# Visual-Behavior/detr-tensorflow

Measured on AMD Instinct MI355X. Metric: images/sec training step, DETR-R50 800x1333 bs=8/GPU, higher is better.
Workload: dtype bf16

## Files before the change

detr-tensorflow_amd/csrc/common.h:

```cpp
#pragma once
#include <hip/hip_runtime.h>
#include <stdint.h>
#include <stdio.h>
#include <stdarg.h>
#include <stdlib.h>

#include "../../include/detr_hip.h"

namespace detr {

void set_error(const char *fmt, ...);

#define DETR_REQUIRE(cond, ...)                 \
    do {                                        \
        if (!(cond)) {                          \
            ::detr::set_error(__VA_ARGS__);     \
            return -1;                          \
        }                                       \
    } while (0)

#define DETR_LAUNCH_CHECK(name)                                                         \
    do {                                                                                \
        hipError_t e__ = hipGetLastError();                                             \
        if (e__ != hipSuccess) {                                                        \
            ::detr::set_error("%s: launch failed: %s", name, hipGetErrorString(e__));   \
            return -2;                                                                  \
        }                                                                               \
    } while (0)

void launch_splitk_reduce(const detr_reduce_desc &r, hipStream_t stream);

constexpr int MIN_WAVES_64X64 = 1;

#if defined(__HIPCC__)
__device__ __forceinline__ void wave_lds_sync() {
    __builtin_amdgcn_fence(__ATOMIC_SEQ_CST, "wavefront");
    __builtin_amdgcn_wave_barrier();
}
__device__ __forceinline__ void lds_barrier() {
    __builtin_amdgcn_fence(__ATOMIC_RELEASE, "workgroup", "local");
    __builtin_amdgcn_s_barrier();
    __builtin_amdgcn_fence(__ATOMIC_ACQUIRE, "workgroup", "local");
}
#endif

enum TuneKey {
    T_GEMM_TILE,
    T_SPLIT_XCD,
    T_GEMM_STREAM,
    T_GEMM_GROUP,
    T_STREAM_SL,
    T_STREAM_NW,
    T_CONV_HALO,
    T_CONV_TILE,
    T_DGRAD_S2_CLASSES,
    T_WGRAD_FUSED,
    T_WGRAD_FUSED_WGS,
    T_WGRAD_TILE,
    T_STEM_ROWS,
    T_ATTN_WAVES,
    T_ATTN_SPLIT,
    T_GEMM_K64,
    T_EPI_WIDE,
    T_SLAB_TS,
    T_GEMM_RING,
// ... 77 lines not shown
```

detr-tensorflow_amd/csrc/optim.hip:

```cpp
#include "common.h"

namespace detr {

__global__ __launch_bounds__(256) void sumsq_segments_kernel(const float *__restrict__ g,
                                                             const int *__restrict__ chunk_tensor,
                                                             const long long *__restrict__ chunk_start,
                                                             const long long *__restrict__ seg_end, int chunk,
                                                             float *__restrict__ sumsq) {
    __shared__ float red[4];
    const int c = blockIdx.x;
    const int t = chunk_tensor[c];
    const long long s0 = chunk_start[c];
    long long s1 = s0 + chunk;
    if (s1 > seg_end[t]) s1 = seg_end[t];
    float acc = 0.f;
    for (long long i = s0 + threadIdx.x; i < s1; i += blockDim.x) {
        const float v = g[i];
        acc += v * v;
    }
    acc = wave_sum(acc);
    if ((threadIdx.x & 63) == 0) red[threadIdx.x >> 6] = acc;
    __syncthreads();
    if (threadIdx.x == 0) sumsq[c] = (red[0] + red[1]) + (red[2] + red[3]);
}

__global__ __launch_bounds__(256) void clip_adam_kernel(float *__restrict__ param, const float *__restrict__ g,
                                                        float *__restrict__ m, float *__restrict__ v,
                                                        const int *__restrict__ chunk_tensor,
                                                        const long long *__restrict__ chunk_start,
                                                        const long long *__restrict__ seg_end,
                                                        const int *__restrict__ tensor_group,
                                                        const float *__restrict__ sumsq,
                                                        const float *__restrict__ hyper, int chunk, int n_chunks) {
    const int c = blockIdx.x;
    const int t = chunk_tensor[c];
    const long long s0 = chunk_start[c];
    long long s1 = s0 + chunk;
    if (s1 > seg_end[t]) s1 = seg_end[t];
    const int grp = tensor_group[t];
    if (grp < 0) return;
    const float lr_t = hyper[grp];
    const float clip = hyper[3], b1 = hyper[4], b2 = hyper[5], eps = hyper[6];
    float cs = 1.0f;
    if (clip > 0.f) {
        __shared__ int s_lo, s_hi;
        __shared__ float s_red[4];
        if (threadIdx.x == 0) {
            int a = 0, b = c;
            while (a < b) { const int mid = (a + b) >> 1; if (chunk_tensor[mid] < t) a = mid + 1; else b = mid; }
            s_lo = a;
            a = c; b = n_chunks;
            while (a < b) { const int mid = (a + b) >> 1; if (chunk_tensor[mid] <= t) a = mid + 1; else b = mid; }
            s_hi = a;
        }
        __syncthreads();
        float acc = 0.f;
        for (int k = s_lo + (int)threadIdx.x; k < s_hi; k += blockDim.x) acc += sumsq[k];
        acc = wave_sum(acc);
        if ((threadIdx.x & 63) == 0) s_red[threadIdx.x >> 6] = acc;
        __syncthreads();
        const float nrm = sqrtf((s_red[0] + s_red[1]) + (s_red[2] + s_red[3]));
        cs = clip / fmaxf(nrm, clip);
    }
    for (long long i = s0 + threadIdx.x; i < s1; i += blockDim.x) {
        const float gi = g[i] * cs;
        const float mi = b1 * m[i] + (1.0f - b1) * gi;
        const float vi = b2 * v[i] + (1.0f - b2) * gi * gi;
        m[i] = mi;
        v[i] = vi;
        param[i] = param[i] - lr_t * mi / (sqrtf(vi) + eps);
    }
}

__global__ void set_floats8_kernel(float *dst, float v0, float v1, float v2, float v3, float v4, float v5, float v6,
                                   float v7) {
    if (threadIdx.x == 0 && blockIdx.x == 0) {
        dst[0] = v0; dst[1] = v1; dst[2] = v2; dst[3] = v3; dst[4] = v4; dst[5] = v5; dst[6] = v6; dst[7] = v7;
    }
}

struct Floats16 { float v[16]; };

__global__ void set_floats16_kernel(float *dst, Floats16 f) {
    if (blockIdx.x == 0 && threadIdx.x < 16) dst[threadIdx.x] = f.v[threadIdx.x];
}
// ... 236 lines not shown
    hipLaunchKernelGGL(set_floats8_kernel, dim3(1), dim3(64), 0, (hipStream_t)stream, dst, v0, v1, v2, v3, v4, v5, v6, v7);
    DETR_LAUNCH_CHECK("set_floats8");
    return 0;
}

extern "C" int detr_hip_sumsq_segments_f32(const float *g, const int32_t *chunk_tensor, const int64_t *chunk_start,
                                           const int64_t *seg_end, int32_t n_chunks, int32_t chunk, float *sumsq,
                                           void *stream) {
    DETR_REQUIRE(g && chunk_tensor && chunk_start && seg_end && sumsq && n_chunks > 0 && chunk > 0, "sumsq: bad args");
    hipLaunchKernelGGL(sumsq_segments_kernel, dim3(n_chunks), dim3(256), 0, (hipStream_t)stream, g, chunk_tensor,
                       reinterpret_cast<const long long *>(chunk_start), reinterpret_cast<const long long *>(seg_end),
                       chunk, sumsq);
    DETR_LAUNCH_CHECK("sumsq_segments");
    return 0;
}

extern "C" int detr_hip_clip_adam_f32(float *param, const float *g, float *m, float *v, const int32_t *chunk_tensor,
                                      const int64_t *chunk_start, const int64_t *seg_end, const int32_t *tensor_group,
                                      const float *sumsq, const float *hyper, int32_t n_chunks, int32_t chunk,
                                      void *stream) {
    DETR_REQUIRE(param && g && m && v && chunk_tensor && chunk_start && seg_end && tensor_group && sumsq && hyper,
                 "clip_adam: null operand");
    DETR_REQUIRE(n_chunks > 0 && chunk > 0, "clip_adam: bad chunking");
    hipLaunchKernelGGL(clip_adam_kernel, dim3(n_chunks), dim3(256), 0, (hipStream_t)stream, param, g, m, v, chunk_tensor,
                       reinterpret_cast<const long long *>(chunk_start), reinterpret_cast<const long long *>(seg_end),
                       tensor_group, sumsq, hyper, chunk, n_chunks);
    DETR_LAUNCH_CHECK("clip_adam");
    return 0;
}
```

detr-tensorflow_amd/csrc/rowops.hip:

```cpp
#include "common.h"

namespace detr {

constexpr int LN_MAXV = 4;

__device__ __forceinline__ unsigned ln_pk_bf16(float a, float b) {
    typedef __bf16 bf16x2_t __attribute__((ext_vector_type(2)));
    bf16x2_t r;
    r[0] = (__bf16)a;
    r[1] = (__bf16)b;
    return __builtin_bit_cast(unsigned, r);
}

__global__ __launch_bounds__(256) void layernorm_fwd_kernel(const float *__restrict__ x, const float *__restrict__ gamma,
                                                            const float *__restrict__ beta, float *__restrict__ y,
                                                            float *__restrict__ mean, float *__restrict__ rstd,
                                                            int rows, int C, float eps, const float *__restrict__ add,
                                                            int add_rows, float *__restrict__ y2, unsigned short *__restrict__ y16) {
    const int lane = threadIdx.x & 63;
    const int wpb = blockDim.x >> 6;
    const int nv = C >> 2;
    for (int row = blockIdx.x * wpb + (threadIdx.x >> 6); row < rows; row += gridDim.x * wpb) {
        const float4 *xr = reinterpret_cast<const float4 *>(x + (long long)row * C);
        float4 v[LN_MAXV];
// ... 303 lines not shown
                     d->dropout_p >= 0.0f && d->dropout_p < 1.0f, "layernorm bwd: dx_drop needs 0 <= p < 1 and aligned outputs");
        drop_scale = d->dropout_p > 0.0f ? 1.0f / (1.0f - d->dropout_p) : 0.0f;
    }
    const int grid = min(cdiv(rows, 8), 512);
    float *partial = (d->workspace && d->workspace_bytes >= (long long)grid * 2 * C * 4) ? d->workspace : nullptr;
    hipLaunchKernelGGL(layernorm_bwd_kernel, dim3(grid), dim3(256), 0, (hipStream_t)stream, d->dy, d->x, d->gamma, d->mean, d->rstd,
                       d->dx, d->dgamma, d->dbeta, rows, C, partial, d->dx_add, d->dx_drop, drop_scale, drop_thresh16(d->dropout_p),
                       d->dropout_site, d->dropout_step, d->dx_drop16, d->dy_add);
    DETR_LAUNCH_CHECK("layernorm bwd");
    if (d->defer_blocks_out) {
        DETR_REQUIRE(partial != nullptr, "layernorm bwd: defer_blocks_out needs a workspace of %d * 2 * C floats", grid);
        *d->defer_blocks_out = grid;
        return 0;
    }
    if (partial) {
        hipLaunchKernelGGL(layernorm_bwd_finish_kernel, dim3(cdiv(2 * C, 64)), dim3(1024), 0, (hipStream_t)stream, partial, grid,
                           C, d->dgamma, d->dbeta);
        DETR_LAUNCH_CHECK("layernorm bwd finish");
    }
    return 0;
}

namespace detr {
typedef __bf16 bf16x2_t __attribute__((ext_vector_type(2)));
__device__ __forceinline__ unsigned pk2_bf16(float a, float b) {
    bf16x2_t r;
    r[0] = (__bf16)a;
    r[1] = (__bf16)b;
    return __builtin_bit_cast(unsigned, r);
}
__global__ void cvt_bf16_kernel(const float4 *__restrict__ x, uint2 *__restrict__ out, long long n4) {
    for (long long i = blockIdx.x * (long long)blockDim.x + threadIdx.x; i < n4; i += (long long)gridDim.x * blockDim.x) {
        const float4 v = x[i];
        out[i] = make_uint2(pk2_bf16(v.x, v.y), pk2_bf16(v.z, v.w));
    }
}
__global__ void scale_cols_bf16_kernel(const float4 *__restrict__ w, const float4 *__restrict__ scale, uint2 *__restrict__ out,
                                       long long n4, int c4) {
    for (long long i = blockIdx.x * (long long)blockDim.x + threadIdx.x; i < n4; i += (long long)gridDim.x * blockDim.x) {
        const float4 v = w[i], sc = scale[i % c4];
        out[i] = make_uint2(pk2_bf16(v.x * sc.x, v.y * sc.y), pk2_bf16(v.z * sc.z, v.w * sc.w));
    }
}

static_assert(sizeof(detr_scale_entry) == 40, "detr_scale_entry layout changed: update Engine._refold_group");

__global__ void scale_cols_bf16_group_kernel(const detr_scale_entry *__restrict__ tab) {
    const detr_scale_entry e = tab[blockIdx.y];
    const float4 *w = reinterpret_cast<const float4 *>(e.w), *scale = reinterpret_cast<const float4 *>(e.scale);
    uint2 *out = reinterpret_cast<uint2 *>(e.out);
    for (long long i = blockIdx.x * (long long)blockDim.x + threadIdx.x; i < e.n4; i += (long long)gridDim.x * blockDim.x) {
        const float4 v = w[i], sc = scale[i % e.c4];
        out[i] = make_uint2(pk2_bf16(v.x * sc.x, v.y * sc.y), pk2_bf16(v.z * sc.z, v.w * sc.w));
// ... 247 lines not shown
```

detr-tensorflow_amd/detr_tf/_hip.py:

```python
import ctypes
import os
from ctypes import POINTER, Structure, byref, c_float, c_int32, c_int64, c_size_t, c_void_p

import torch

_HERE = os.path.dirname(os.path.abspath(__file__))
LIB_PATH = os.environ.get("DETR_HIP_LIB") or os.path.join(os.path.dirname(_HERE), "lib", "libdetr_hip.so")

f32p = c_void_p


class ReduceDesc(Structure):
    _fields_ = [("ws", c_void_p), ("splits", c_int32), ("part_stride", c_int64), ("rows", c_int32), ("cols", c_int32),
                ("C", c_void_p), ("ldc", c_int64), ("alpha", c_float), ("scale", c_void_p),
                ("rs_ws", c_void_p), ("rs_out", c_void_p), ("rs_alpha", c_float),
                ("ts_bm", c_int32), ("ts_bn", c_int32), ("ts_tiles_n", c_int32)]


class GemmDesc(Structure):
    _fields_ = [("M", c_int32), ("N", c_int32), ("K", c_int32),
                ("A", c_void_p), ("lda", c_int64), ("a_kcontig", c_int32),
                ("B", c_void_p), ("ldb", c_int64), ("b_kcontig", c_int32),
                ("C", c_void_p), ("ldc", c_int64),
                ("batch", c_int32), ("batch_inner", c_int32),
# ... 249 lines not shown
    "detr_hip_add_f32": [f32p, f32p, f32p, c_int64, c_void_p],
    "detr_hip_sigmoid_bwd_f32": [f32p, f32p, f32p, c_int64, c_void_p],
    "detr_hip_relu_mask_f32": [f32p, f32p, f32p, c_int64, c_void_p],
    "detr_hip_scale_cols_f32": [f32p, f32p, f32p, c_int64, c_int32, c_void_p],
    "detr_hip_scale_cols_t_f32": [f32p, f32p, f32p, c_int32, c_int32, c_void_p],
    "detr_hip_bn_fold_f32": [f32p, f32p, f32p, f32p, f32p, f32p, c_int32, c_float, c_void_p],
    "detr_hip_postprocess": [POINTER(PostprocessDesc), c_void_p],
    "detr_hip_map_match": [POINTER(MapMatchDesc), c_void_p],
    "detr_hip_input_stage": [POINTER(InputDesc), c_void_p],
    "detr_hip_pad_labels": [c_void_p, c_void_p, c_void_p, c_int32, c_int32, c_void_p, c_void_p, c_void_p],
    "detr_hip_augment": [c_void_p, c_int64, c_void_p, f32p, c_int32, c_int32, c_int32, f32p, c_void_p, f32p, c_void_p],
    "detr_hip_augment_padded": [c_void_p, c_int64, c_void_p, c_int32, c_int32, c_int32, f32p, c_void_p, f32p, c_void_p, c_void_p],
    "detr_hip_match_cost_f32": [POINTER(SetLossDesc), f32p, c_void_p],
    "detr_hip_assign_f32": [f32p, c_int32, c_int32, c_int32, f32p, c_int32, c_int32, c_void_p, c_void_p, c_void_p, c_void_p],
    "detr_hip_set_loss_sums_f32": [POINTER(SetLossDesc), c_void_p, f32p, c_void_p],
    "detr_hip_set_loss_finalize_f32": [f32p, c_int32, f32p, f32p, c_void_p],
    "detr_hip_set_loss_grad_f32": [POINTER(SetLossDesc), c_void_p, f32p, c_float, f32p, f32p, c_void_p],
    "detr_hip_match_cost_crit_f32": [POINTER(SetLossDesc), POINTER(c_float), f32p, c_void_p],
    "detr_hip_set_loss_sums_crit_f32": [POINTER(SetLossDesc), POINTER(c_float), f32p, c_void_p, f32p, c_void_p],
    "detr_hip_set_loss_finalize_crit_f32": [f32p, c_int32, POINTER(c_float), f32p, f32p, c_void_p],
    "detr_hip_set_loss_grad_crit_f32": [POINTER(SetLossDesc), POINTER(c_float), f32p, c_void_p, f32p, c_float, f32p, f32p, c_void_p],
    "detr_hip_sumsq_segments_f32": [f32p, c_void_p, c_void_p, c_void_p, c_int32, c_int32, f32p, c_void_p],
    "detr_hip_clip_adam_f32": [f32p, f32p, f32p, f32p, c_void_p, c_void_p, c_void_p, c_void_p, f32p, f32p, c_int32, c_int32, c_void_p],
    "detr_hip_axpy_f32": [f32p, f32p, c_float, c_int64, c_void_p],
    "detr_hip_set_floats8_f32": [f32p] + [c_float] * 8 + [c_void_p],
    "detr_hip_set_floats16_f32": [f32p, POINTER(c_float * 16), c_void_p],
    "detr_hip_global_clip_scale_f32": [f32p, c_void_p, c_void_p, f32p, c_int32, f32p, c_void_p],
    "detr_hip_adamw_f32": [f32p, f32p, f32p, f32p, c_void_p, c_void_p, c_void_p, c_void_p, f32p, f32p, f32p, c_int32, c_int32, c_void_p],
    "detr_hip_ema_f32": [f32p, f32p, c_void_p, c_void_p, c_void_p, f32p, c_int32, c_int32, c_void_p],
    "detr_hip_exchange_f32": [f32p, f32p, c_int64, c_void_p],
    "detr_hip_conv3x3_dilated": [POINTER(Conv3x3DDesc), c_int32, c_void_p],
    "detr_hip_detect": [POINTER(DetectDesc), c_void_p],
    "detr_hip_tile_merge": [POINTER(TileMergeDesc), c_void_p],
    "detr_hip_coco_match": [POINTER(CocoMatchDesc), c_void_p],
    "detr_hip_overlay": [POINTER(OverlayDesc), c_void_p],
    "detr_hip_track": [POINTER(TrackDesc), c_void_p],
    "detr_hip_track_embed": [POINTER(TrackEmbedDesc), c_void_p],
    "detr_hip_track_motion": [POINTER(TrackMotionDesc), c_void_p],
    "detr_hip_fuse_views": [POINTER(TileMergeDesc), c_void_p, POINTER(ctypes.c_double * FUSE_PARAMS), c_void_p, c_void_p],
}
_SIGNATURES_I64 = {
    "detr_hip_attention_dropmask_words": [c_int32, c_int32, c_int32, c_int32],
    "detr_hip_attention_keymask_words": [c_int32, c_int32],
    "detr_hip_colsum_det_scratch_floats": [c_int64, c_int32],
    "detr_hip_conv1x1_bwd_fused_workspace_floats": [c_int64],
    "detr_hip_workspace_bytes_gemm": [POINTER(GemmDesc)],
# ... 717 lines not shown
```

detr-tensorflow_amd/detr_tf/engine.py:

```python
import math
import os
from ctypes import byref, c_float
from typing import NamedTuple, Optional

import numpy as np
import torch

from . import _hip as hip
from .params import ParamStore, RESNET50_BLOCKS, block_names, bn_conv_pairs, stem_names
from .streams import DropMasks, SideStream

D = 256
HEADS = 8
HD = 32
FF = 2048
BN_EPS = 1e-5
KERAS_BN_EPS = 1.001e-5
LN_EPS = 1e-5
DEFER_REDUCE = os.environ.get("DETR_HIP_DEFER_REDUCE", "1") != "0"
WGRAD_STREAM = os.environ.get("DETR_HIP_WGRAD_STREAM", "1") != "0"
BWD_FUSED = os.environ.get("DETR_HIP_BWD_FUSED", "1") != "0"
DROPMASK_AHEAD = int(os.environ.get("DETR_HIP_DROPMASK_AHEAD", "2") or 0)
QK_ALPHA = float(HD) ** -0.5 * 1.4426950408889634

# ... 107 lines not shown
        if DEFER_REDUCE:
            hip.ensure_defer_workspace(self.device)
        self.blocks = tuple(blocks)
        self.num_enc, self.num_dec, self.Q = num_enc, num_dec, num_queries
        self.nb_class = nb_class
        self.C = num_classes if nb_class is None else nb_class
        self.tf_backbone = bool(tf_backbone)
        self.bn_eps = KERAS_BN_EPS if self.tf_backbone else BN_EPS
        self.P = ParamStore(self.device, blocks, num_enc, num_dec, num_queries, num_classes, nb_class, seed, tf_backbone=tf_backbone)
        self._stem = stem_names(self.tf_backbone)
        self._pairs = bn_conv_pairs(self.blocks, self.tf_backbone)
        self._bufs = {}
        self._buf_gen = 0
        self._pos_cache = {}
        self._pos_tables = {}
        self.key_valid = None
        self._attn_sites = ()
        self.attn_maps = {}
        self._shape = None
        self._adt = torch.float32
        self._block_recs = []
        self._feat_meta = None
        self._fold_table = self._shift_table = None
        self.bn_scale, self.bn_shift = {}, {}
        self._weights_version, self._built = 0, {}
        self.P.on_change = self._params_changed
        self.fold_bn()
        self.compute = 0
        self.f32_split = False
        self.dropout_p = 0.1
        self.dropout_seed = 0x5EED
        self.dp_rank = 0
        self._step_no = 0
        self._drop = (0.0, 0)
        self._step_seed = 0
        self._seed_dev = torch.zeros(8, dtype=torch.int32, device=self.device)
        self._cross = {}
        self._graph_replay = False
        self.phase_events = None
        self.side = SideStream(self.device)
        self.masks = DropMasks(self, HEADS)

    @property
    def gemm_mode(self):
        return 1 if self.compute == 1 else (2 if self.f32_split else 0)

    def bump_weights_version(self):
        self._weights_version += 1

    def _stale(self, key):
        if self._built.get(key) == self._weights_version:
            return False
        self._built[key] = self._weights_version
        return True

    def seed_of_step(self, step_no):
        return step_seed(self.dropout_seed, step_no, self.dp_rank)

    def advance_dropout_step(self):
        self._step_no += 1
        self._step_seed = self.seed_of_step(self._step_no)
        self.masks.settle()
        hip.call("detr_hip_set_u32x8", self._seed_dev.data_ptr(), self._step_seed, self.seed_of_step(self._step_no + 1),
                 0, 0, 0, 0, 0, 0)
        self._drop = (float(self.dropout_p), self._step_seed)
        return self._step_seed

    def phase(self, name):
        if self.phase_events is not None:
            ev = torch.cuda.Event(enable_timing=True)
            ev.record()
# ... 48 lines not shown

    def _w(self, name):
        if self.compute == 1 and self.P.views16 is not None:
            return self.P.views16[name]
        return self.P.views[name]

    def _refresh_shadow(self):
        flat16 = self.P.shadow16()
        hip.call("detr_hip_cvt_bf16", self.P.flat.data_ptr(), flat16.data_ptr(), self.P.flat.numel())
        self._refold_group()

    def _refold_group(self):
        if self._fold_table is None:
            rows = []
            for bn_name, conv in self._pairs[1:]:
                conv_name = f"{conv}/kernel"
                w = self.P.views[conv_name]
                co = w.shape[-1]
                ws16 = self.buf(f"ws16:{conv_name}", w.shape, torch.bfloat16)
                rows.append([w.data_ptr(), self.bn_scale[bn_name].data_ptr(), ws16.data_ptr(), w.numel() // 4, co // 4])
            self._fold_table = torch.tensor(rows, dtype=torch.int64).to(self.device)
            self._fold_keep = [self.bn_scale, self._bufs]
        hip.call("detr_hip_scale_cols_bf16_group", self._fold_table.data_ptr(), self._fold_table.shape[0])

    def _scaled_kernel(self, conv_name, bn_name):
        w = self.P.views[conv_name]
        co = w.shape[-1]
        if self.compute == 1 and conv_name != f"{self._stem['conv']}/kernel":
            return self.buf(f"ws16:{conv_name}", w.shape, torch.bfloat16)
        ws = self.buf(f"ws:{conv_name}", w.shape)
        if self._stale(f"ws:{conv_name}"):
            hip.call("detr_hip_scale_cols_f32", w.data_ptr(), self.bn_scale[bn_name].data_ptr(), ws.data_ptr(),
                     w.numel() // co, co)
        return ws

    def _conv1x1_fwd(self, x, M, cin, cout, conv_name, bn_name, out, residual=None, act=1, maskbits_out=None):
        ws = self._scaled_kernel(conv_name, bn_name)
        shift = self.bn_shift[bn_name]
        ldr = cout if residual is not None else 0
        hip.gemm(M, cout, cin, x, cin, 1, ws, cout, 0, out, cout, bias=shift, residual=residual, ldr=ldr, act=act,
                 maskbits_out=maskbits_out)

    @staticmethod
    def _wgrad(M_out, N_out, K_red, A, lda, Bm, ldb, C, ldc, scale=None, alpha=1.0, compute=None):
        sk = hip.pick_split_k(M_out, N_out, K_red, compute=compute)
        if sk > 1:
# ... 749 lines not shown
```

detr-tensorflow_amd/detr_tf/optimizers.py:

```python
import math
from ctypes import byref, c_float

import numpy as np
import torch

from . import _hip as hip
from .params import GROUPS

CHUNK = 8192


class GroupAdam:

    def __init__(self, store, group_id, lr_getter, clipnorm, nlayers, engine=None, config=None):
        self.store, self.group_id, self.lr_getter, self.clipnorm = store, group_id, lr_getter, clipnorm
        self.config = config
        self.engine = engine
        self.iterations = 0
        self.beta_1, self.beta_2, self.epsilon = 0.9, 0.999, 1e-7
        dev = store.device
        tables = store.build_tables(nlayers, CHUNK)
        grp = tables["group_host"]
        keep = [i for i, t in enumerate(tables["chunk_tensor"].tolist()) if grp[t] == group_id]
        self.names = [n for n, g in zip(tables["names"], grp) if g == group_id]
        self.n_chunks = len(keep)
        idx = torch.tensor(keep, dtype=torch.int64, device=dev)
        self.chunk_tensor = tables["chunk_tensor"][idx].contiguous() if keep else None
        self.chunk_start = tables["chunk_start"][idx].contiguous() if keep else None
        self.seg_end = tables["seg_end"]
        self.tensor_group = torch.tensor(grp, dtype=torch.int32, device=dev)
        self.sumsq = torch.zeros(max(1, self.n_chunks), dtype=torch.float32, device=dev)
        if not hasattr(store, "adam_m"):
            store.adam_m = torch.zeros_like(store.flat)
            store.adam_v = torch.zeros_like(store.flat)
        self.m, self.v = store.adam_m, store.adam_v
        self.hyper = torch.zeros(16, dtype=torch.float32, device=dev)

    def learning_rate(self):
        return float(self.lr_getter())

    def weight_decay(self):
# ... 1 lines not shown

    def step_sizes(self):
        t, lr = self.iterations, self.learning_rate()
        return lr, lr * math.sqrt(1.0 - self.beta_2 ** t) / (1.0 - self.beta_1 ** t)

    def set_step_hyper(self):
        self.iterations += 1
        t = self.iterations
        self.epsilon = float(getattr(self.config, "adam_epsilon", self.epsilon))
        lr_t = self.learning_rate() * math.sqrt(1.0 - self.beta_2 ** t) / (1.0 - self.beta_1 ** t)
        clip = self.clipnorm if self.clipnorm is not None else 0.0
        wd = self.weight_decay()
        if wd > 0.0:
            lr = self.learning_rate()
            write_hyper16(self.hyper, [lr_t, lr_t, lr_t, clip, self.beta_1, self.beta_2, self.epsilon, wd, lr, lr, lr, 1.0, 1.0, 1.0,
                                       0.0, 0.0])
            return
        hip.call("detr_hip_set_floats8_f32", self.hyper.data_ptr(), lr_t, lr_t, lr_t, clip, self.beta_1, self.beta_2,
                 self.epsilon, 0.0)

    def apply_gradients(self, grad_flat, hyper_ready=False):
        if not hyper_ready:
            self.set_step_hyper()
        if self.engine is not None:
            self.engine.bump_weights_version()
        if self.n_chunks == 0:
            return
        hip.call("detr_hip_sumsq_segments_f32", grad_flat.data_ptr(), self.chunk_tensor.data_ptr(),
                 self.chunk_start.data_ptr(), self.seg_end.data_ptr(), self.n_chunks, CHUNK, self.sumsq.data_ptr())
        if self.weight_decay() > 0.0:
            hip.call("detr_hip_adamw_f32", self.store.flat.data_ptr(), grad_flat.data_ptr(), self.m.data_ptr(), self.v.data_ptr(),
                     self.chunk_tensor.data_ptr(), self.chunk_start.data_ptr(), self.seg_end.data_ptr(), self.tensor_group.data_ptr(),
                     self.sumsq.data_ptr(), self.hyper.data_ptr(), None, self.n_chunks, CHUNK)
            return
        hip.call("detr_hip_clip_adam_f32", self.store.flat.data_ptr(), grad_flat.data_ptr(), self.m.data_ptr(),
                 self.v.data_ptr(), self.chunk_tensor.data_ptr(), self.chunk_start.data_ptr(), self.seg_end.data_ptr(),
                 self.tensor_group.data_ptr(), self.sumsq.data_ptr(), self.hyper.data_ptr(), self.n_chunks, CHUNK)


def write_hyper16(dst, values):
    hip.call("detr_hip_set_floats16_f32", dst.data_ptr(), byref((c_float * 16)(*[float(x) for x in values])))


def clip_mode(config):
    return "joint" if getattr(config, "global_clipnorm", None) is not None else "tensor"


def decay_active(config):
    return float(getattr(config, "weight_decay", 0.0) or 0.0) > 0.0


def trained_groups(config):
    return [n for n in GROUPS if getattr(config, f"train_{n}")]


def trained_chunk_table(tables, group_host, trained, device, cache):
# ... 242 lines not shown
    if ema_active(config):
        weight_ema(optimizers, config).prepare()
    if clip_mode(config) == "joint":
        joint = joint_optimizer(optimizers, config)
        last = name == trained_groups(config)[-1]
        if gradient_aggregate is None or gradient_aggregate <= 1:
            optimizers[gname] = store.grad
            if last:
                joint.apply(store.grad)
                applied(name, optimizers, config)
            return
        acc = optimizers[gname] = joint.accumulator(optimizers)
        for a, b in joint.runs[opt.group_id]:
            if step % gradient_aggregate == 0:
                hip.call("detr_hip_memset_zero", acc.data_ptr() + 4 * a, 4 * (b - a))
            hip.call("detr_hip_axpy_f32", acc.data_ptr() + 4 * a, store.grad.data_ptr() + 4 * a, c_float(1.0), b - a)
        if last and (step + 1) % gradient_aggregate == 0:
            joint.apply(acc)
            applied(name, optimizers, config)
        return
    if gradient_aggregate is None or gradient_aggregate <= 1:
        optimizers[gname] = store.grad
        opt.apply_gradients(store.grad)
        applied(name, optimizers, config)
        return
    acc = optimizers.get(gname)
    if not isinstance(acc, torch.Tensor) or acc is store.grad or acc is optimizers.get("_joint_gradients"):
        acc = optimizers[gname] = torch.zeros_like(store.grad)
    elif step % gradient_aggregate == 0:
        hip.zero_(acc)
    for n in opt.names:
        o, cnt = store.offsets[n]
        hip.call("detr_hip_axpy_f32", acc.data_ptr() + 4 * o, store.grad.data_ptr() + 4 * o, c_float(1.0), cnt)
    if (step + 1) % gradient_aggregate == 0:
        opt.apply_gradients(acc)
        applied(name, optimizers, config)


def applied(name, optimizers, config):
    model_dirty(optimizers)
    if ema_active(config) and name == trained_groups(config)[-1]:
        weight_ema(optimizers, config).apply()


def model_dirty(optimizers):
    eng = optimizers.get("_engine")
    if eng is not None:
        eng.bump_weights_version()


def optimizer_state(optimizers):
    store = optimizers["_store"]
    _in_ema_scope(store, "optimizer_state")
    m, v = store.adam_m.cpu().numpy(), store.adam_v.cpu().numpy()
    out = {}
    for k, (o, n) in store.offsets.items():
        out[f"m/{k}"] = m[o:o + n].reshape(store.shapes[k]).copy()
        out[f"v/{k}"] = v[o:o + n].reshape(store.shapes[k]).copy()
    for name in GROUPS:
        opt = optimizers[f"{name}_optimizer"]
        out[f"iterations/{name}"] = np.asarray(opt.iterations, dtype=np.int64)
        acc = optimizers.get(f"{name}_gradients")
        if isinstance(acc, torch.Tensor) and acc is not store.grad:
            host = acc.cpu().numpy()
            for k in opt.names:
                o, n = store.offsets[k]
                out[f"accum/{k}"] = host[o:o + n].reshape(store.shapes[k]).copy()
    eng = optimizers.get("_engine")
    if eng is not None:
        out["engine/step_no"] = np.asarray(eng._step_no, dtype=np.int64)
    if getattr(store, "ema", None) is not None:
# ... 84 lines not shown
```

detr-tensorflow_amd/detr_tf/training.py:

```python
import contextlib
import gc
import os
import time

import numpy as np
import torch

from . import _hip as hip
from .engine import downsample_mask_nearest, feature_size
from .loss import hungarian_matching as _matching
from .loss.loss import criterion_of, get_losses, log_from_losses
from .optimizers import (GROUPS, aggregate_grad_and_apply, clip_mode, decay_active, ema_active, ema_weights, gather_gradient,
                         joint_optimizer, weight_ema)

PRINT_EVERY_TRAIN = 100
PRINT_EVERY_VAL = 10


def _gradient_aggregate(config):
    if config.target_batch is not None:
        return max(1, int(config.target_batch // config.batch_size))
    return 1


def run_train_step(model, images, t_bbox, t_class, optimizers, config):
    gradient_aggregate = _gradient_aggregate(config)
    optimizers["_engine"] = model.engine
    m_outputs = model(images, training=True)
    _matching.before_assign = model.engine.pregen_dropmasks_at_matcher
    try:
        total_loss, log = get_losses(m_outputs, t_bbox, t_class, config)
    finally:
        _matching.before_assign = None
    total_loss = total_loss / gradient_aggregate
    gradient_steps = gather_gradient(model, optimizers, total_loss, m_outputs, config, log,
                                     loss_scale=1.0 / gradient_aggregate)
# ... 52 lines not shown

    def replay(self):
        for g, act in zip(self.graphs, self.actions):
            g.replay()
            if act is not None:
                act()


class GraphedTrainStep:

    PROBE_STEPS = 3

    def __init__(self, model, optimizers, config, eager_steps=1, launch="graph"):
        assert launch in ("graph", "eager", "auto")
        self.model, self.optimizers, self.config = model, optimizers, config
        self.eager_steps = max(1, int(eager_steps))
        self.launch = launch
        self.calls = 0
        self.key = None
        self.step_graph = self.apply_graph = None
        self.static = None
        self.result = None
        self._gen = -1
        self.choice = "eager" if launch == "eager" else "graph"
        self.probe = None
        self._probe_t = {}
        self._probe_dirty = False
        self._probe_skipped = False
        self.total_calls = 0

    def _signature(self, images, t_bbox, t_class):
        c = self.config
        images, masks = split_images(images)
        return (tuple(images.shape), masks is not None, tuple(t_bbox.shape), bool(c.train_backbone), bool(c.train_transformers),
                bool(c.train_nlayers), int(c.background_class), self.model.engine.compute, float(self.model.engine.dropout_p),
                bool(getattr(c, "check_matching", False)), clip_mode(c), decay_active(c), ema_active(c), tuple(self.model.engine.dilate),
                criterion_of(c))

    def _capture(self, images, t_bbox, t_class):
        model, opts, cfg = self.model, self.optimizers, self.config
        eng, dev = model.engine, model.device
        img, masks = split_images(images)
        st_img = torch.empty(tuple(img.shape), dtype=torch.float32, device=dev)
        st_tb = torch.empty(tuple(t_bbox.shape), dtype=torch.float32, device=dev)
        st_tc = torch.empty((t_bbox.shape[0], t_bbox.shape[1]), dtype=torch.int64, device=dev)
        st_mask = torch.empty(tuple(masks.shape), dtype=torch.uint8, device=dev) if masks is not None else None
        self.static = (st_img, st_tb, st_tc, st_mask)
        self._load_inputs(images, t_bbox, t_class)
        dp = model.dp
        if clip_mode(cfg) == "joint":
            joint_optimizer(opts, cfg).prepare()
        if ema_active(cfg):
            weight_ema(opts, cfg).prepare()
        seg = _Segments()
        side = torch.cuda.Stream(device=dev)
        side.wait_stream(torch.cuda.current_stream())
        eng._graph_replay = True
        eng.bump_weights_version()
        prev_hooks = None
        gc_was_on = gc.isenabled()
        gc.collect()
        gc.disable()
        try:
            with torch.cuda.stream(side):
                if dp is not None and dp.active:
                    prev_hooks = (dp.on_bucket, dp.reduce_sums, dp.finish)
                    dp.on_bucket = lambda i, f=prev_hooks[0]: seg.cut(lambda: f(i))
                    dp.reduce_sums = lambda sums, f=prev_hooks[1]: seg.cut(lambda: f(sums))
                    dp.finish = lambda: None
                seg.begin()
                m_outputs, total_loss, log, gradient_steps = run_train_step(model, st_img if st_mask is None else (st_img, st_mask),
                                                                            st_tb, st_tc, opts, cfg)
                seg.end()
                if prev_hooks is not None:
                    dp.on_bucket, dp.reduce_sums, dp.finish = prev_hooks
                    prev_hooks = None
                app = _Segments()
                app.pool = seg.pool
                app.begin()
                store = opts["_store"]
                joint = clip_mode(cfg) == "joint"
                for name in GROUPS:
                    if getattr(cfg, f"train_{name}"):
                        opts[f"{name}_gradients"] = store.grad
                        if not joint:
                            opts[f"{name}_optimizer"].apply_gradients(store.grad, hyper_ready=True)
                if joint:
                    joint_optimizer(opts, cfg).apply(store.grad, hyper_ready=True)
                if ema_active(cfg):
                    weight_ema(opts, cfg).apply(hyper_ready=True)
                app.end()
        finally:
            if prev_hooks is not None:
                dp.on_bucket, dp.reduce_sums, dp.finish = prev_hooks
            eng._graph_replay = False
            if gc_was_on:
                gc.enable()
        torch.cuda.current_stream().wait_stream(side)
        self.step_graph, self.apply_graph = seg, app
        self.result = (m_outputs, m_outputs.set_loss)
        self._gen = eng.buf_generation

    def _load_inputs(self, images, t_bbox, t_class):
        st_img, st_tb, st_tc, st_mask = self.static
        images, masks = split_images(images)
        if st_mask is not None:
            if not (torch.is_tensor(masks) and masks.is_cuda):
                host = np.asarray(masks.cpu() if torch.is_tensor(masks) else masks).astype(bool)
                Hf, Wf = feature_size(host.shape[1], host.shape[2], self.model.engine.dilate)
                empty = [b for b in range(host.shape[0]) if downsample_mask_nearest(host[b:b + 1], Hf, Wf).all()]
                if empty:
                    raise ValueError(f"masks: image(s) {empty} have no valid (unpadded) position on the {Hf} x {Wf} feature map")
                masks = torch.from_numpy(host.view(np.uint8))
            if not (torch.is_tensor(masks) and masks.data_ptr() == st_mask.data_ptr()):
                st_mask.copy_(torch.as_tensor(masks).to(torch.uint8), non_blocking=True)
        if not (torch.is_tensor(images) and images.data_ptr() == st_img.data_ptr()):
            st_img.copy_(torch.as_tensor(images), non_blocking=True)
        if not (torch.is_tensor(t_bbox) and t_bbox.data_ptr() == st_tb.data_ptr()):
            st_tb.copy_(torch.as_tensor(t_bbox), non_blocking=True)
        tc = torch.as_tensor(t_class)
        if not (tc.is_cuda and tc.data_ptr() == st_tc.data_ptr()):
            st_tc.copy_(tc.reshape(st_tc.shape), non_blocking=True)

    def _replay(self, images, t_bbox, t_class):
        cfg, model = self.config, self.model
        if self.step_graph is None:
            self._capture(images, t_bbox, t_class)
        else:
            self._load_inputs(images, t_bbox, t_class)
        eng = model.engine
        eng._graph_replay = True
        try:
            if eng.dropout_p > 0.0:
                eng.advance_dropout_step()
            if clip_mode(cfg) == "joint":
                joint_optimizer(self.optimizers, cfg).set_step_hyper()
            else:
                for name in GROUPS:
                    if getattr(cfg, f"train_{name}"):
                        self.optimizers[f"{name}_optimizer"].set_step_hyper()
            if ema_active(cfg):
                weight_ema(self.optimizers, cfg).set_step_hyper()
            self.step_graph.replay()
            if model.dp is not None:
                model.dp.finish()
            self.apply_graph.replay()
        finally:
            eng._graph_replay = False
        eng.bump_weights_version()
        m_outputs, sl = self.result
        log = log_from_losses(sl.losses.clone())
        total_loss = sl.total.clone()[0]
        for name in GROUPS:
            log[f"{name}_lr"] = self.optimizers[f"{name}_optimizer"].learning_rate()
        return m_outputs, total_loss, log

    def _decide(self):
        n = self.PROBE_STEPS
        tg, te = self._probe_t.get("graph_s"), self._probe_t.get("eager_s")
        tg = float("inf") if tg is None else tg
        te = float("inf") if te is None else te
        dp = self.model.dp
        if dp is not None and getattr(dp, "active", False):
            import torch.distributed as dist
            big = 1.0e30
            tt = torch.tensor([min(tg, big), min(te, big)], dtype=torch.float64, device=self.model.device)
            dist.all_reduce(tt, op=dist.ReduceOp.MAX, group=getattr(dp, "group", None))
            tg, te = (float(v) for v in tt.tolist())
            tg = float("inf") if tg >= big else tg
            te = float("inf") if te >= big else te
        self.choice = "graph" if (tg != float("inf") and te != float("inf") and tg <= te) else "eager"
        ms = lambda t: None if t == float("inf") else round(t / n * 1e3, 3)
# ... 120 lines not shown
```

include/detr_hip.h:

```cpp
#ifndef DETR_HIP_H
#define DETR_HIP_H

#include <stddef.h>
#include <stdint.h>

#ifdef __cplusplus
extern "C" {
#endif

#define DETR_HIP_ABI_VERSION 9

const char *detr_hip_last_error(void);
int detr_hip_abi_version(void);
int detr_hip_reload_tuning(void);
int detr_hip_struct_layout(int32_t which, int32_t *out, int32_t cap);
int detr_hip_memset_zero(void *ptr, size_t bytes, void *stream);

typedef struct detr_reduce_desc {
    const float *ws; int32_t splits; int64_t part_stride; int32_t rows, cols;
    float *C; int64_t ldc; float alpha; const float *scale;
    const float *rs_ws; float *rs_out; float rs_alpha;
    int32_t ts_bm, ts_bn, ts_tiles_n;
} detr_reduce_desc;

// ... 256 lines not shown
    int64_t sD_b;
    const float *t_bbox;  int64_t sT_b;
    const int64_t *t_class; int64_t sC_b;
    double thresholds[DETR_MAP_MAX_THR];
    float *rec_score;
    int32_t *rec_class;
    uint32_t *rec_flags;
    int64_t *num_gt;
    int32_t *status;
} detr_map_match_desc;
int detr_hip_map_match(const detr_map_match_desc *d, void *stream);

int detr_hip_sumsq_segments_f32(const float *g, const int32_t *chunk_tensor, const int64_t *chunk_start,
                                const int64_t *seg_end, int32_t n_chunks, int32_t chunk, float *sumsq,
                                void *stream);
int detr_hip_clip_adam_f32(float *param, const float *g, float *m, float *v, const int32_t *chunk_tensor,
                           const int64_t *chunk_start, const int64_t *seg_end, const int32_t *tensor_group,
                           const float *sumsq, const float *hyper, int32_t n_chunks, int32_t chunk,
                           void *stream);
int detr_hip_set_floats8_f32(float *dst, float v0, float v1, float v2, float v3, float v4, float v5, float v6,
                             float v7, void *stream);
int detr_hip_axpy_f32(float *acc, const float *g, float a, int64_t n, void *stream);

int detr_hip_set_floats16_f32(float *dst, const float *values, void *stream);
int detr_hip_global_clip_scale_f32(const float *sumsq, const int32_t *chunk_tensor, const int32_t *tensor_group,
                                   const float *hyper, int32_t n_chunks, float *scale, void *stream);
int detr_hip_adamw_f32(float *param, const float *g, float *m, float *v, const int32_t *chunk_tensor,
                       const int64_t *chunk_start, const int64_t *seg_end, const int32_t *tensor_group,
                       const float *sumsq, const float *hyper, const float *scale, int32_t n_chunks, int32_t chunk,
                       void *stream);

int detr_hip_ema_f32(float *shadow, const float *param, const int32_t *chunk_tensor, const int64_t *chunk_start,
                     const int64_t *seg_end, const float *hyper, int32_t n_chunks, int32_t chunk, void *stream);
int detr_hip_exchange_f32(float *a, float *b, int64_t n, void *stream);

int64_t detr_hip_workspace_bytes_gemm(const detr_gemm_desc *d);
int64_t detr_hip_workspace_bytes_conv3x3(const detr_conv3x3_desc *d, int32_t mode);
int64_t detr_hip_workspace_bytes_stem(const detr_stem_desc *d, int32_t mode);
int64_t detr_hip_workspace_bytes_layernorm(const detr_layernorm_desc *d);

int detr_hip_gemm_ring_plan(int32_t M, int32_t N, int32_t K, int32_t *out);

typedef struct {
    int32_t N, Hi, Wi, Ci, Ho, Wo, Co, stride, pad;
    const float *x;
    const float *w;
// ... 243 lines not shown
```

Before: 522.4.

## Fuse bf16 shadow-weight refresh into clip-Adam update kernel

Adds a templated clip-Adam kernel that, after updating fp32 params, also writes the bf16 shadow copy, applying the folded BN column scale for conv kernels. The engine then marks the shadow as current instead of rebuilding it on the next forward. This removes a separate pass that re-reads all fp32 params to regenerate bf16 and BN-folded weights. It also vectorizes the update with float4. The cost is a more complex version-tracking protocol and a path limited to configs without weight decay, joint clipping, or non-power-of-two output channels.

```diff
diff --git a/detr-tensorflow_amd/csrc/common.h b/detr-tensorflow_amd/csrc/common.h
--- a/detr-tensorflow_amd/csrc/common.h
+++ b/detr-tensorflow_amd/csrc/common.h
@@ -41,6 +41,13 @@
     __builtin_amdgcn_fence(__ATOMIC_RELEASE, "workgroup", "local");
     __builtin_amdgcn_s_barrier();
     __builtin_amdgcn_fence(__ATOMIC_ACQUIRE, "workgroup", "local");
+}
+typedef __bf16 bf16x2_t __attribute__((ext_vector_type(2)));
+__device__ __forceinline__ unsigned pk2_bf16(float a, float b) {
+    bf16x2_t r;
+    r[0] = (__bf16)a;
+    r[1] = (__bf16)b;
+    return __builtin_bit_cast(unsigned, r);
 }
 #endif
 
diff --git a/detr-tensorflow_amd/csrc/optim.hip b/detr-tensorflow_amd/csrc/optim.hip
--- a/detr-tensorflow_amd/csrc/optim.hip
+++ b/detr-tensorflow_amd/csrc/optim.hip
@@ -24,6 +24,18 @@
     if (threadIdx.x == 0) sumsq[c] = (red[0] + red[1]) + (red[2] + red[3]);
 }
 
+__device__ __forceinline__ float clip_adam_elem(float p, float gi, float &m, float &v, float cs, float b1, float b2,
+                                                float eps, float lr_t) {
+#pragma clang fp contract(off)
+    gi = gi * cs;
+    const float mi = b1 * m + (1.0f - b1) * gi;
+    const float vi = b2 * v + (1.0f - b2) * gi * gi;
+    m = mi;
+    v = vi;
+    return p - lr_t * mi / (sqrtf(vi) + eps);
+}
+
+template <bool SHADOW>
 __global__ __launch_bounds__(256) void clip_adam_kernel(float *__restrict__ param, const float *__restrict__ g,
                                                         float *__restrict__ m, float *__restrict__ v,
                                                         const int *__restrict__ chunk_tensor,
@@ -31,7 +43,8 @@
                                                         const long long *__restrict__ seg_end,
                                                         const int *__restrict__ tensor_group,
                                                         const float *__restrict__ sumsq,
-                                                        const float *__restrict__ hyper, int chunk, int n_chunks) {
+                                                        const float *__restrict__ hyper, int chunk, int n_chunks,
+                                                        const detr_shadow_entry *__restrict__ shadow) {
     const int c = blockIdx.x;
     const int t = chunk_tensor[c];
     const long long s0 = chunk_start[c];
@@ -61,6 +74,52 @@
         __syncthreads();
         const float nrm = sqrtf((s_red[0] + s_red[1]) + (s_red[2] + s_red[3]));
         cs = clip / fmaxf(nrm, clip);
+    }
+    if constexpr (SHADOW) {
+        const detr_shadow_entry e = shadow[t];
+        const long long j0 = s0 - e.start;
+        uint16_t *__restrict__ out = e.out ? e.out + j0 : nullptr;
+        const float *__restrict__ scale = e.scale;
+        const long long cmask = e.cols - 1;
+        long long i0 = s0;
+        const uintptr_t bufs = (uintptr_t)param | (uintptr_t)g | (uintptr_t)m | (uintptr_t)v;
+        if ((bufs & 15) == 0 && (s0 & 3) == 0 && ((uintptr_t)out & 7) == 0 &&
+            (!scale || (((uintptr_t)scale & 15) == 0 && (j0 & 3) == 0 && (e.cols & 3) == 0))) {
+            const long long nvec = (s1 - s0) >> 2;
+            float4 *__restrict__ p4 = reinterpret_cast<float4 *>(param + s0);
+            float4 *__restrict__ m4 = reinterpret_cast<float4 *>(m + s0);
+            float4 *__restrict__ v4 = reinterpret_cast<float4 *>(v + s0);
+            const float4 *__restrict__ g4 = reinterpret_cast<const float4 *>(g + s0);
+            uint2 *__restrict__ out4 = reinterpret_cast<uint2 *>(out);
+            for (long long j = threadIdx.x; j < nvec; j += blockDim.x) {
+                const float4 gg = g4[j];
+                float4 pp = p4[j], mm = m4[j], vv = v4[j];
+                pp.x = clip_adam_elem(pp.x, gg.x, mm.x, vv.x, cs, b1, b2, eps, lr_t);
+                pp.y = clip_adam_elem(pp.y, gg.y, mm.y, vv.y, cs, b1, b2, eps, lr_t);
+                pp.z = clip_adam_elem(pp.z, gg.z, mm.z, vv.z, cs, b1, b2, eps, lr_t);
+                pp.w = clip_adam_elem(pp.w, gg.w, mm.w, vv.w, cs, b1, b2, eps, lr_t);
+                m4[j] = mm;
+                v4[j] = vv;
+                p4[j] = pp;
+                if (out) {
+                    if (scale) {
+                        const float4 sc = *reinterpret_cast<const float4 *>(scale + ((j0 + 4 * j) & cmask));
+                        pp.x *= sc.x; pp.y *= sc.y; pp.z *= sc.z; pp.w *= sc.w;
+                    }
+                    out4[j] = make_uint2(pk2_bf16(pp.x, pp.y), pk2_bf16(pp.z, pp.w));
+                }
+            }
+            i0 = s0 + (nvec << 2);
+        }
+        for (long long i = i0 + threadIdx.x; i < s1; i += blockDim.x) {
+            float mi = m[i], vi = v[i];
+            const float pn = clip_adam_elem(param[i], g[i], mi, vi, cs, b1, b2, eps, lr_t);
+            m[i] = mi;
+            v[i] = vi;
+            param[i] = pn;
+            if (out) out[i - s0] = (uint16_t)pk2_bf16(scale ? pn * scale[(i - e.start) & cmask] : pn, 0.f);
+        }
+        return;
     }
     for (long long i = s0 + threadIdx.x; i < s1; i += blockDim.x) {
         const float gi = g[i] * cs;
@@ -343,9 +402,24 @@
     DETR_REQUIRE(param && g && m && v && chunk_tensor && chunk_start && seg_end && tensor_group && sumsq && hyper,
                  "clip_adam: null operand");
     DETR_REQUIRE(n_chunks > 0 && chunk > 0, "clip_adam: bad chunking");
-    hipLaunchKernelGGL(clip_adam_kernel, dim3(n_chunks), dim3(256), 0, (hipStream_t)stream, param, g, m, v, chunk_tensor,
+    hipLaunchKernelGGL(clip_adam_kernel<false>, dim3(n_chunks), dim3(256), 0, (hipStream_t)stream, param, g, m, v, chunk_tensor,
                        reinterpret_cast<const long long *>(chunk_start), reinterpret_cast<const long long *>(seg_end),
-                       tensor_group, sumsq, hyper, chunk, n_chunks);
+                       tensor_group, sumsq, hyper, chunk, n_chunks, (const detr_shadow_entry *)nullptr);
     DETR_LAUNCH_CHECK("clip_adam");
     return 0;
 }
+
+extern "C" int detr_hip_clip_adam_shadow_f32(float *param, const float *g, float *m, float *v, const int32_t *chunk_tensor,
+                                             const int64_t *chunk_start, const int64_t *seg_end, const int32_t *tensor_group,
+                                             const float *sumsq, const float *hyper, int32_t n_chunks, int32_t chunk,
+                                             const detr_shadow_entry *shadow, void *stream) {
+    DETR_REQUIRE(param && g && m && v && chunk_tensor && chunk_start && seg_end && tensor_group && sumsq && hyper,
+                 "clip_adam_shadow: null operand");
+    DETR_REQUIRE(shadow, "clip_adam_shadow: null shadow table (detr_hip_clip_adam_f32 is the call without one)");
+    DETR_REQUIRE(n_chunks > 0 && chunk > 0, "clip_adam_shadow: bad chunking");
+    hipLaunchKernelGGL(clip_adam_kernel<true>, dim3(n_chunks), dim3(256), 0, (hipStream_t)stream, param, g, m, v, chunk_tensor,
+                       reinterpret_cast<const long long *>(chunk_start), reinterpret_cast<const long long *>(seg_end),
+                       tensor_group, sumsq, hyper, chunk, n_chunks, shadow);
+    DETR_LAUNCH_CHECK("clip_adam_shadow");
+    return 0;
+}
diff --git a/detr-tensorflow_amd/csrc/rowops.hip b/detr-tensorflow_amd/csrc/rowops.hip
--- a/detr-tensorflow_amd/csrc/rowops.hip
+++ b/detr-tensorflow_amd/csrc/rowops.hip
@@ -349,13 +349,6 @@
 }
 
 namespace detr {
-typedef __bf16 bf16x2_t __attribute__((ext_vector_type(2)));
-__device__ __forceinline__ unsigned pk2_bf16(float a, float b) {
-    bf16x2_t r;
-    r[0] = (__bf16)a;
-    r[1] = (__bf16)b;
-    return __builtin_bit_cast(unsigned, r);
-}
 __global__ void cvt_bf16_kernel(const float4 *__restrict__ x, uint2 *__restrict__ out, long long n4) {
     for (long long i = blockIdx.x * (long long)blockDim.x + threadIdx.x; i < n4; i += (long long)gridDim.x * blockDim.x) {
         const float4 v = x[i];
diff --git a/detr-tensorflow_amd/detr_tf/_hip.py b/detr-tensorflow_amd/detr_tf/_hip.py
--- a/detr-tensorflow_amd/detr_tf/_hip.py
+++ b/detr-tensorflow_amd/detr_tf/_hip.py
@@ -295,6 +295,8 @@
     "detr_hip_set_loss_grad_crit_f32": [POINTER(SetLossDesc), POINTER(c_float), f32p, c_void_p, f32p, c_float, f32p, f32p, c_void_p],
     "detr_hip_sumsq_segments_f32": [f32p, c_void_p, c_void_p, c_void_p, c_int32, c_int32, f32p, c_void_p],
     "detr_hip_clip_adam_f32": [f32p, f32p, f32p, f32p, c_void_p, c_void_p, c_void_p, c_void_p, f32p, f32p, c_int32, c_int32, c_void_p],
+    "detr_hip_clip_adam_shadow_f32": [f32p, f32p, f32p, f32p, c_void_p, c_void_p, c_void_p, c_void_p, f32p, f32p, c_int32, c_int32, c_void_p,
+                                      c_void_p],
     "detr_hip_axpy_f32": [f32p, f32p, c_float, c_int64, c_void_p],
     "detr_hip_set_floats8_f32": [f32p] + [c_float] * 8 + [c_void_p],
     "detr_hip_set_floats16_f32": [f32p, POINTER(c_float * 16), c_void_p],
diff --git a/detr-tensorflow_amd/detr_tf/engine.py b/detr-tensorflow_amd/detr_tf/engine.py
--- a/detr-tensorflow_amd/detr_tf/engine.py
+++ b/detr-tensorflow_amd/detr_tf/engine.py
@@ -153,6 +153,8 @@
         self._block_recs = []
         self._feat_meta = None
         self._fold_table = self._shift_table = None
+        self._adam_table = None
+        self.adam_writes_shadow = True
         self.bn_scale, self.bn_shift = {}, {}
         self._weights_version, self._built = 0, {}
         self.P.on_change = self._params_changed
@@ -176,8 +178,11 @@
     def gemm_mode(self):
         return 1 if self.compute == 1 else (2 if self.f32_split else 0)
 
-    def bump_weights_version(self):
+    def bump_weights_version(self, shadow_written=False):
+        keep = shadow_written and self._built.get("shadow16") == self._weights_version
         self._weights_version += 1
+        if keep:
+            self._built["shadow16"] = self._weights_version
 
     def _stale(self, key):
         if self._built.get(key) == self._weights_version:
@@ -272,6 +277,33 @@
             self._fold_table = torch.tensor(rows, dtype=torch.int64).to(self.device)
             self._fold_keep = [self.bn_scale, self._bufs]
         hip.call("detr_hip_scale_cols_bf16_group", self._fold_table.data_ptr(), self._fold_table.shape[0])
+
+    def shadow_table(self):
+        if not (self.adam_writes_shadow and self.compute == 1 and self.P.views16 is not None
+                and self._built.get("shadow16") == self._weights_version):
+            return None
+        if self._adam_table is None:
+            folded = {f"{conv}/kernel": bn_name for bn_name, conv in self._pairs[1:]}
+            rows = []
+            for k, (o, _) in self.P.offsets.items():
+                bn_name = folded.get(k)
+                if bn_name is None:
+                    rows.append([self.P.flat16.data_ptr() + 2 * o, 0, o, 1])
+                    continue
+                co = self.P.shapes[k][-1]
+                if co & (co - 1):
+                    self._adam_table = False
+                    return None
+                rows.append([self._bufs[f"ws16:{k}"].data_ptr(), self.bn_scale[bn_name].data_ptr(), o, co])
+            self._adam_table = torch.tensor(rows, dtype=torch.int64).to(self.device)
+        return self._adam_table if self._adam_table is not False else None
+
+    def prepare_adam_shadow(self):
+        if not (self.adam_writes_shadow and self.compute == 1):
+            return False
+        if self._stale("shadow16") or self.P.views16 is None:
+            self._refresh_shadow()
+        return self.shadow_table() is not None
 
     def _scaled_kernel(self, conv_name, bn_name):
         w = self.P.views[conv_name]
diff --git a/detr-tensorflow_amd/detr_tf/optimizers.py b/detr-tensorflow_amd/detr_tf/optimizers.py
--- a/detr-tensorflow_amd/detr_tf/optimizers.py
+++ b/detr-tensorflow_amd/detr_tf/optimizers.py
@@ -17,6 +17,7 @@
         self.config = config
         self.engine = engine
         self.iterations = 0
+        self.wrote_shadow = False
         self.beta_1, self.beta_2, self.epsilon = 0.9, 0.999, 1e-7
         dev = store.device
         tables = store.build_tables(nlayers, CHUNK)
@@ -64,8 +65,11 @@
     def apply_gradients(self, grad_flat, hyper_ready=False):
         if not hyper_ready:
             self.set_step_hyper()
-        if self.engine is not None:
-            self.engine.bump_weights_version()
+        table = None
+        if hasattr(self.engine, "shadow_table") and self.weight_decay() <= 0.0:
+            table = self.engine.shadow_table()
+        self.wrote_shadow = table is not None
+        weights_moved(self.engine, self.wrote_shadow)
         if self.n_chunks == 0:
             return
         hip.call("detr_hip_sumsq_segments_f32", grad_flat.data_ptr(), self.chunk_tensor.data_ptr(),
@@ -74,6 +78,12 @@
             hip.call("detr_hip_adamw_f32", self.store.flat.data_ptr(), grad_flat.data_ptr(), self.m.data_ptr(), self.v.data_ptr(),
                      self.chunk_tensor.data_ptr(), self.chunk_start.data_ptr(), self.seg_end.data_ptr(), self.tensor_group.data_ptr(),
                      self.sumsq.data_ptr(), self.hyper.data_ptr(), None, self.n_chunks, CHUNK)
+            return
+        if table is not None:
+            hip.call("detr_hip_clip_adam_shadow_f32", self.store.flat.data_ptr(), grad_flat.data_ptr(), self.m.data_ptr(),
+                     self.v.data_ptr(), self.chunk_tensor.data_ptr(), self.chunk_start.data_ptr(), self.seg_end.data_ptr(),
+                     self.tensor_group.data_ptr(), self.sumsq.data_ptr(), self.hyper.data_ptr(), self.n_chunks, CHUNK,
+                     table.data_ptr())
             return
         hip.call("detr_hip_clip_adam_f32", self.store.flat.data_ptr(), grad_flat.data_ptr(), self.m.data_ptr(),
                  self.v.data_ptr(), self.chunk_tensor.data_ptr(), self.chunk_start.data_ptr(), self.seg_end.data_ptr(),
@@ -362,7 +372,7 @@
     if gradient_aggregate is None or gradient_aggregate <= 1:
         optimizers[gname] = store.grad
         opt.apply_gradients(store.grad)
-        applied(name, optimizers, config)
+        applied(name, optimizers, config, shadow_written=opt.wrote_shadow)
         return
     acc = optimizers.get(gname)
     if not isinstance(acc, torch.Tensor) or acc is store.grad or acc is optimizers.get("_joint_gradients"):
@@ -374,19 +384,24 @@
         hip.call("detr_hip_axpy_f32", acc.data_ptr() + 4 * o, store.grad.data_ptr() + 4 * o, c_float(1.0), cnt)
     if (step + 1) % gradient_aggregate == 0:
         opt.apply_gradients(acc)
-        applied(name, optimizers, config)
-
-
-def applied(name, optimizers, config):
-    model_dirty(optimizers)
+        applied(name, optimizers, config, shadow_written=opt.wrote_shadow)
+
+
+def applied(name, optimizers, config, shadow_written=False):
+    model_dirty(optimizers, shadow_written)
     if ema_active(config) and name == trained_groups(config)[-1]:
         weight_ema(optimizers, config).apply()
 
 
-def model_dirty(optimizers):
-    eng = optimizers.get("_engine")
-    if eng is not None:
-        eng.bump_weights_version()
+def model_dirty(optimizers, shadow_written=False):
+    weights_moved(optimizers.get("_engine"), shadow_written)
+
+
+def weights_moved(engine, shadow_written=False):
+    if engine is not None and shadow_written:
+        engine.bump_weights_version(shadow_written=True)
+    elif engine is not None:
+        engine.bump_weights_version()
 
 
 def optimizer_state(optimizers):
diff --git a/detr-tensorflow_amd/detr_tf/training.py b/detr-tensorflow_amd/detr_tf/training.py
--- a/detr-tensorflow_amd/detr_tf/training.py
+++ b/detr-tensorflow_amd/detr_tf/training.py
@@ -11,7 +11,7 @@
 from .loss import hungarian_matching as _matching
 from .loss.loss import criterion_of, get_losses, log_from_losses
 from .optimizers import (GROUPS, aggregate_grad_and_apply, clip_mode, decay_active, ema_active, ema_weights, gather_gradient,
-                         joint_optimizer, weight_ema)
+                         joint_optimizer, weight_ema, weights_moved)
 
 PRINT_EVERY_TRAIN = 100
 PRINT_EVERY_VAL = 10
@@ -110,6 +110,7 @@
         self.static = None
         self.result = None
         self._gen = -1
+        self._tail_shadow = False
         self.choice = "eager" if launch == "eager" else "graph"
         self.probe = None
         self._probe_t = {}
@@ -123,6 +124,7 @@
         return (tuple(images.shape), masks is not None, tuple(t_bbox.shape), bool(c.train_backbone), bool(c.train_transformers),
                 bool(c.train_nlayers), int(c.background_class), self.model.engine.compute, float(self.model.engine.dropout_p),
                 bool(getattr(c, "check_matching", False)), clip_mode(c), decay_active(c), ema_active(c), tuple(self.model.engine.dilate),
+                bool(getattr(self.model.engine, "adam_writes_shadow", False)),
                 criterion_of(c))
 
     def _capture(self, images, t_bbox, t_class):
@@ -141,10 +143,11 @@
         if ema_active(cfg):
             weight_ema(opts, cfg).prepare()
         seg = _Segments()
+        eng.bump_weights_version()
+        self._tail_shadow = clip_mode(cfg) != "joint" and not decay_active(cfg) and eng.prepare_adam_shadow()
         side = torch.cuda.Stream(device=dev)
         side.wait_stream(torch.cuda.current_stream())
         eng._graph_replay = True
-        eng.bump_weights_version()
         prev_hooks = None
         gc_was_on = gc.isenabled()
         gc.collect()
@@ -185,6 +188,8 @@
             if gc_was_on:
                 gc.enable()
         torch.cuda.current_stream().wait_stream(side)
+        if self._tail_shadow:
+            assert all(opts[f"{name}_optimizer"].wrote_shadow for name in GROUPS if getattr(cfg, f"train_{name}"))
         self.step_graph, self.apply_graph = seg, app
         self.result = (m_outputs, m_outputs.set_loss)
         self._gen = eng.buf_generation
@@ -229,13 +234,15 @@
                         self.optimizers[f"{name}_optimizer"].set_step_hyper()
             if ema_active(cfg):
                 weight_ema(self.optimizers, cfg).set_step_hyper()
+            if self._tail_shadow:
+                eng.prepare_adam_shadow()
             self.step_graph.replay()
             if model.dp is not None:
                 model.dp.finish()
             self.apply_graph.replay()
         finally:
             eng._graph_replay = False
-        eng.bump_weights_version()
+        weights_moved(eng, self._tail_shadow)
         m_outputs, sl = self.result
         log = log_from_losses(sl.losses.clone())
         total_loss = sl.total.clone()[0]
diff --git a/include/detr_hip.h b/include/detr_hip.h
--- a/include/detr_hip.h
+++ b/include/detr_hip.h
@@ -302,6 +302,18 @@
                              float v7, void *stream);
 int detr_hip_axpy_f32(float *acc, const float *g, float a, int64_t n, void *stream);
 
+typedef struct detr_shadow_entry {
+    uint16_t *out;
+    const float *scale;
+    int64_t start;
+    int32_t cols;
+    int32_t reserved;
+} detr_shadow_entry;
+int detr_hip_clip_adam_shadow_f32(float *param, const float *g, float *m, float *v, const int32_t *chunk_tensor,
+                                  const int64_t *chunk_start, const int64_t *seg_end, const int32_t *tensor_group,
+                                  const float *sumsq, const float *hyper, int32_t n_chunks, int32_t chunk,
+                                  const detr_shadow_entry *shadow, void *stream);
+
 int detr_hip_set_floats16_f32(float *dst, const float *values, void *stream);
 int detr_hip_global_clip_scale_f32(const float *sumsq, const int32_t *chunk_tensor, const int32_t *tensor_group,
                                    const float *hyper, int32_t n_chunks, float *scale, void *stream);
```

Result: no change. 525.4, median of 6 (+0.6%).
